# rvp-group/srrg2_slam_interfaces

Hardware: AMD Instinct MI355X
Metric: icp_iterations_per_sec (higher is better)
Workload: dtype f32; 1 GPU; C2: SE(3) point-to-plane AlignerSlice, 100000-pt synthetic cloud pair per GPU, 10 ICP iterations per compute(), gated NN 0.25 m + normal gate, Cauchy 0.05; points=100000, alignments_total=1, all_success=True, last_status=0, last_num_inliers=99432, parallelism=single GPU

## Files before the change

include/srrg2_slam_amd.h:

```cpp
#ifndef SRRG2_SLAM_AMD_H
#define SRRG2_SLAM_AMD_H

#include <stddef.h>
#include <stdint.h>

#ifdef __cplusplus
extern "C" {
#endif

#define SRRG2_AMD_ABI_VERSION 4
#define SRRG2_MAX_SLICES 8


enum srrg2_variable_kind {
  SRRG2_SE2_RIGHT       = 0,
  SRRG2_SE3_EULER_RIGHT = 1,
  SRRG2_SE3_QUAT_RIGHT  = 2
};

enum srrg2_status {
  SRRG2_SUCCESS                    = 0,
  SRRG2_NOT_ENOUGH_CORRESPONDENCES = 1,
  SRRG2_NOT_ENOUGH_INLIERS         = 2,
  SRRG2_FAIL                       = 3
// ... 390 lines not shown
  float   rmax_cap;
  int32_t search_lists;
  int32_t search_team;
  int32_t batch_pipeline;
  int32_t fused_control;
  int32_t reserved_[6];
} srrg2_aligner_tuning;
void srrg2_aligner_default_tuning(srrg2_aligner_tuning* t);
int srrg2_aligner_get_tuning(srrg2_aligner_h h, srrg2_aligner_tuning* t_out);
int srrg2_aligner_set_tuning(srrg2_aligner_h h, const srrg2_aligner_tuning* t);


int srrg2_aligner_profile_enable(srrg2_aligner_h h, int enable);
int srrg2_aligner_profile_get(srrg2_aligner_h h, double* step_kernel_ms, int64_t* step_kernel_launches,
                              int reset);
#define SRRG2_PATH_FUSED_CONTROL 1
#define SRRG2_PATH_ALL_PASSES_FUSED 2
#define SRRG2_PATH_FINAL_WAVE 4
#define SRRG2_PATH_PROLOGUE_IN_PASS 8
#define SRRG2_PATH_ONE_WORKGROUP 16
#define SRRG2_PATH_PRIORS_FUSED 32
int srrg2_aligner_last_compute_path(srrg2_aligner_h h, int32_t* flags_out);

#ifndef SRRG2_DESCRIPTOR_BYTES
#define SRRG2_DESCRIPTOR_BYTES 32
#endif
typedef struct srrg2_descriptor_db* srrg2_descriptor_db_h;
int srrg2_descriptor_db_create(int device, srrg2_descriptor_db_h* out);
int srrg2_descriptor_db_destroy(srrg2_descriptor_db_h h);
int srrg2_descriptor_db_add(srrg2_descriptor_db_h h, const uint8_t* descriptors, const uint8_t* valid, int n,
                            int* index_out);
int srrg2_descriptor_db_size(srrg2_descriptor_db_h h, int* maps, int64_t* descriptors);
int srrg2_descriptor_db_match(srrg2_descriptor_db_h h, const uint8_t* descriptors, const uint8_t* valid, int n,
                              int64_t query_index, float max_distance, uint32_t min_age, int64_t min_matches,
                              int* K_out);
int srrg2_descriptor_db_get_candidates(srrg2_descriptor_db_h h, int32_t* reference, int64_t* num_matches,
                                       int64_t* corr_offsets, int* n_inout);
int srrg2_descriptor_db_get_correspondences(srrg2_descriptor_db_h h, srrg2_correspondence* buf, int64_t* n_inout);
int srrg2_descriptor_db_get_map_counts(srrg2_descriptor_db_h h, int64_t* counts, int* n_inout);
int srrg2_descriptor_db_last_match_ms(srrg2_descriptor_db_h h, double* ms);
int srrg2_descriptor_db_add_scene(srrg2_descriptor_db_h h, srrg2_scene_h scene, int* index_out);
int srrg2_descriptor_db_match_scene(srrg2_descriptor_db_h h, srrg2_scene_h scene, int64_t query_index, float max_distance,
                                    uint32_t min_age, int64_t min_matches, int* K_out);

#ifdef __cplusplus
}
// ... 3 lines not shown
```

srrg2_slam_interfaces_amd/csrc/aligner_host.hip:

```cpp
#include <algorithm>
#include <cmath>
#include <cstdio>
#include <cstdlib>
#include <chrono>
#include <cstring>
#include <string>
#include <vector>

#include "det_math.h"
#include "kernels.h"

#include "host_util.h"

namespace srrg2amd {
thread_local std::string g_err;
int fail(int code, const std::string& msg) {
  g_err = msg;
  return code;
}
}

namespace {

using srrg2amd::DevBuf;
using srrg2amd::fail;

struct Slice {
  srrg2_slice_config cfg;
  DevBuf<float4> fixed_raw, fixed_nrm_raw;
  DevBuf<float4> fixed_sorted, fixed_nrm_sorted;
  DevBuf<int> cell_start, cursor, scan_sums, pos_of;
  DevBuf<unsigned> scalars;
  GridDev grid{};
  DevBuf<int> list_start, list_sums;
  DevBuf<uint4> list_ent;
  DevBuf<uint2> list_box;
  DevBuf<int4> list_offs;
  DevBuf<GridLists> list_hdr;
  GridLists lists_host{};
  bool lists_tried = false;
  int grid_computes = 0;
  int nf          = 0;
  float probe_h = 0.f, probe_ext = 0.f, probe_gate = 0.f, probe_target = 0.f;
  int probe_n   = 0;
  bool has_fixed  = false;
  bool fixed_has_normals = false;
  int alias_of = -1;
  DevBuf<float4> moving, moving_nrm;
  DevBuf<float4> moving_raw, moving_nrm_raw;
  DevBuf<int> ms_counts, ms_cursor, ms_sums;
  DevBuf<unsigned> ms_bb;
  DevBuf<ProblemDev> ms_probs;
  DevBuf<unsigned> pinf;
  int nm_total            = 0;
  bool has_moving         = false;
  bool moving_is_batch    = false;
  bool moving_has_normals = false;
  DevBuf<int> corr_fixed;
// ... 17 lines not shown
  const void* slots_zeroed_at = nullptr;
  int slots_zeroed = 0;
  unsigned* bbox_host = nullptr; size_t bbox_host_cap = 0;
  unsigned bbox_seq = 0;
  bool scalars_self_init = false;
  DevBuf<unsigned> bbox_rows;
  DevBuf<unsigned long long> zbuf;
  DevBuf<int> queue;
  DevBuf<int> qcount;
  float prior_Z[12]{};
  bool has_prior = false;
  void release() {
    if (qprobe_host) (void) hipHostFree(qprobe_host);
    qprobe_host = nullptr;
    qprobe_cap  = 0;
    if (bbox_host) (void) hipHostFree(bbox_host);
    bbox_host     = nullptr;
    bbox_host_cap = 0;
    if (ms_probs_host) (void) hipHostFree(ms_probs_host);
    ms_probs_host     = nullptr;
    ms_probs_host_cap = 0;
    fixed_raw.release(); fixed_nrm_raw.release(); fixed_sorted.release(); fixed_nrm_sorted.release();
    cell_start.release(); cursor.release(); scan_sums.release(); scalars.release(); pos_of.release();
    list_start.release(); list_sums.release(); list_ent.release(); list_box.release(); list_offs.release(); list_hdr.release();
    moving.release(); moving_nrm.release(); pinf.release();
    moving_raw.release(); moving_nrm_raw.release(); ms_counts.release(); ms_cursor.release(); ms_sums.release();
    ms_bb.release(); ms_probs.release();
    corr_fixed.release(); gcorr.release(); gcorr_off.release(); gcorr_stat.release(); prev_n.release(); prev_pos.release(); prev_f.release(); prev_m.release(); corr_resp.release(); corr_stat.release(); partials.release(); zbuf.release(); queue.release(); qcount.release(); bbox_rows.release();
  }
};

}

struct srrg2_aligner_s {
  int kind = 0, dim = 3, dof = 6, tsize = 12, device = 0;
  hipStream_t stream = nullptr;
  static constexpr int MAX_PARTS = 8;
  hipStream_t pstream[MAX_PARTS]{};
  int cu_count          = 256;
  int fused_grid_max    = 130000;
  hipEvent_t ev_staged  = nullptr;
  hipEvent_t ev_records = nullptr;
  bool records_unsynced = false;
  int parts_dirty       = 0;
  int batch_parts       = 0;
  int part_begin[MAX_PARTS + 1]{};
  srrg2_aligner_params params{10, 10, 0, 0};
// ... 381 lines not shown
        const int m = sep(x) + sep(y) + sep(z);
        if (m > CNL_MAX_CLASS || class_bound2(m) > g.gate2_ext) continue;
        offs.push_back(Off{x, y, z, m, x * x + y * y + z * z});
      }
  if ((long long) offs.size() * ((long long) s->nf + s->nf / CNL_ENTRY_MAX + 1) >= (1LL << 31)) return 0;
  std::stable_sort(offs.begin(), offs.end(), [](const Off& p, const Off& q) { return p.cls != q.cls ? p.cls < q.cls : p.c2 < q.c2; });
  std::vector<int4> offs4(offs.size());
  for (size_t k = 0; k < offs.size(); ++k) offs4[k] = make_int4(offs[k].x, offs[k].y, offs[k].z, offs[k].cls);
  GridLists L{};
  L.R   = R;
  L.lnx = g.nx + 2 * R;
  L.lny = g.ny + 2 * R;
  L.lnz = dim == 3 ? g.nz + 2 * R : 1;
  const long long ncell_ll = (long long) L.lnx * L.lny * L.lnz;
  if (ncell_ll > (1LL << 28)) return 0;
  const int ncell = (int) ncell_ll;
  for (int m = 0; m <= CNL_MAX_CLASS; ++m) L.cls_b2[m] = class_bound2(m);
  L.cls_b2[CNL_MAX_CLASS + 1] = 3.0e38f;
  int rc;
  if ((rc = s->list_offs.reserve(offs4.size()))) return rc;
  if ((rc = s->list_start.reserve((size_t) ncell + 1))) return rc;
  if ((rc = s->list_sums.reserve((size_t) srrg2amd::scan_num_blocks(ncell) + 2))) return rc;
  if ((rc = s->list_hdr.reserve(1))) return rc;
  HIP_TRY(hipMemcpyAsync(s->list_offs.p, offs4.data(), offs4.size() * sizeof(int4), hipMemcpyHostToDevice, a->stream));
  HIP_TRY(hipStreamSynchronize(a->stream));
  srrg2amd::launch_cnl_build(g, L, s->list_offs.p, (int) offs4.size(), s->list_start.p, nullptr, nullptr, a->stream);
  int* total_dev = s->list_sums.p + s->list_sums.cap - 1;
  srrg2amd::launch_exclusive_scan(s->list_start.p, ncell, s->list_sums.p, total_dev, a->stream);
  int total = 0;
  HIP_TRY(hipMemcpyAsync(&total, total_dev, sizeof(int), hipMemcpyDeviceToHost, a->stream));
  HIP_TRY(hipStreamSynchronize(a->stream));
  if (total < 0 || (long long) total > max_entries) return 0;
  if (s->list_ent.reserve((size_t) std::max(total, 1) + 8) || s->list_box.reserve((size_t) std::max(s->nf, 1) + 8)) {
    (void) hipGetLastError();
    s->list_ent.release();
    s->list_box.release();
    return 0;
  }
  L.start = s->list_start.p;
  L.ent   = s->list_ent.p;
  srrg2amd::launch_cnl_build(g, L, s->list_offs.p, (int) offs4.size(), s->list_start.p, s->list_box.p, s->list_ent.p, a->stream);
  HIP_TRY(hipMemcpyAsync(s->list_hdr.p, &L, sizeof(L), hipMemcpyHostToDevice, a->stream));
  HIP_TRY(hipGetLastError());
  HIP_TRY(hipStreamSynchronize(a->stream));
  g.lists       = s->list_hdr.p;
  g.list_R      = R;
  s->lists_host = L;
  return 0;
}

void tuning_from_environment(srrg2_aligner_tuning* t) {
  srrg2_aligner_default_tuning(t);
  auto geti = [](const char* name, int32_t& v) {
    if (const char* e = std::getenv(name)) v = (int32_t) std::atoi(e);
  };
  auto getf = [](const char* name, float& v) {
    if (const char* e = std::getenv(name)) v = (float) std::atof(e);
  };
  geti("SRRG2_AMD_TUNE", t->strategy_mask);
  geti("SRRG2_AMD_QPROBE", t->queue_probe_iteration);
  geti("SRRG2_AMD_SMALL_MAX", t->small_max_points);
  geti("SRRG2_AMD_FAST_FROM", t->fast_from_iteration);
  geti("SRRG2_AMD_FAST_PPT", t->fast_points_per_thread);
  geti("SRRG2_AMD_FAST_MIN", t->fast_min_points);
// ... 1944 lines not shown
int srrg2_aligner_profile_enable(srrg2_aligner_h a, int enable) {
  if (!a) return fail(SRRG2_E_INVALID, "profile_enable: null handle");
  a->profile = enable != 0;
  return 0;
}

int srrg2_aligner_profile_get(srrg2_aligner_h a, double* ms, int64_t* launches, int reset) {
  if (!a) return fail(SRRG2_E_INVALID, "profile_get: null handle");
  if (ms) *ms = a->prof_ms;
  if (launches) *launches = a->prof_launches;
  if (reset) {
    a->prof_ms       = 0.0;
    a->prof_launches = 0;
  }
  return 0;
}

int srrg2_aligner_last_compute_path(srrg2_aligner_h a, int32_t* flags_out) {
  if (!a || !flags_out) return fail(SRRG2_E_INVALID, "last_compute_path: null argument");
  *flags_out = a->computed ? a->last_path : 0;
  return 0;
}

}
```

srrg2_slam_interfaces_amd/csrc/device_types.h:

```cpp
#pragma once
#include <hip/hip_runtime.h>
#include <stdint.h>

#include "../../include/srrg2_slam_amd.h"

#define ACC_N 32
#define PARTIAL_SLOTS 32
#define ACC_B 21
#define ACC_CHI_IN 27
#define ACC_CHI_OUT 28
#define ACC_N_IN 29
#define ACC_N_OUT 30
#define ACC_N_CORR 31
#define TERM_WINDOW_MAX 64
#define NO_MATCH 0x7fffffff

__host__ __device__ __forceinline__ constexpr int hidx(int a, int b) {
  return a * 6 - (a * (a - 1)) / 2 + (b - a);
}

struct GridDev {
  float ox, oy, oz;
  float h, inv_h;
  int nx, ny, nz;
  int rmax;
  int rfar_gate;
  float gate2;
  float gate2_ext;
  int n;
  const int* cell_start;
  const float4* pts;
  const float4* nrm;
  const int* pos_of;
  int list_R;
  const struct GridLists* lists;
};
struct GridLists {
  int R;
  int lnx, lny, lnz;
  const int* start;
  const uint4* ent;
  float cls_b2[14];
};
#define CNL_MAX_R 3
#ifndef CNL_ENTRY_MAX
#define CNL_ENTRY_MAX 16
#endif
#define CNL_MAX_CLASS 12

#define PUB_SLICE_GRANULES 64
#define PUB_G_KEXP 24
#define PUB_G_FLAGS 25
#define PUB_G_NSTATS 26
#define PUB_G_WCOUNT 27
#define PUB_G_NPASSES 28
#define PUB_G_X 32
#define PUB_FLAG_STOP 1u
#define PUB_FLAG_PHASE1 2u
#define PUB_FLAG_PRIOR 4u
#define PUB_EPOCH_REPLICAS 8
#define PUB_EPOCH_STRIDE 32
struct CtlParams;
struct FusedCtl {
  unsigned long long* pub;
  unsigned* pub_epoch;
  const CtlParams* ctl;
// ... 150 lines not shown
```

srrg2_slam_interfaces_amd/csrc/kernels.h:

```cpp
#pragma once
#include "device_types.h"

namespace srrg2amd {

void launch_ingest(const float* src, int stride_floats, int n, int dim, float4* dst, unsigned* maxabs_bits,
                   int finite_per_point, hipStream_t s);
void launch_ingest_batch(const float* src, int stride_floats, const ProblemDev* probs, int K, int max_nm, int dim,
                         float4* dst, unsigned* maxabs_bits, int finite_per_point, hipStream_t s);
void launch_bbox(const float4* pts, int n, unsigned* mn, unsigned* mx, int* nvalid, hipStream_t s);
void launch_ingest_bbox(const float* src, int stride_floats, int n, int dim, float4* dst, unsigned* maxabs_bits, unsigned* mn,
                        unsigned* mx, int* nvalid, hipStream_t s, unsigned* ticket, unsigned* host_out, unsigned seq,
                        unsigned* block_out , unsigned* clear_after);
#define INGEST_BBOX_MAX_BLOCKS 512
void launch_grid_count(const GridDev& g, const float4* pts, int n, int* counts, hipStream_t s);
void launch_count_nonzero(const int* counts, int n, int* out, hipStream_t s);
int scan_num_blocks(int n);
void launch_exclusive_scan(int* data, int n, int* block_sums, int* grand_total, hipStream_t s, int* copy = nullptr);
void launch_grid_scatter(const GridDev& g, const float4* pts, const float4* nrm, int n, int* cursor, float4* out_pts,
                         float4* out_nrm, int* pos_of, hipStream_t s);
void launch_cnl_build(const GridDev& g, const GridLists& L, const int4* offs, int noffs, int* list_start, uint2* box_at,
                      uint4* ent, hipStream_t s);
void launch_icp_step_cnl(int dim, bool plane, const SliceDev& S, const GridLists& GL, const ProblemDev* probs,
                         ProblemState* states, int K, int max_nm, int team, hipStream_t s, const CtlParams* init_C = nullptr,
                         const InitInline* init_inl = nullptr, const InitBatch* init_bat = nullptr);
bool launch_msort_local(const float* src, int sf, const float* nsrc, int nsf, const ProblemDev* probs, int K, int dim, int kbits,
                        int aniso, int segments, int max_nm, float4* out_pts, float4* out_nrm, unsigned* maxabs_bits,
                        hipStream_t s);
void launch_msort(const float4* pts, const float4* nrm, const ProblemDev* probs, int K, int max_nm, int kbits, int aniso,
                  unsigned* bb, int* counts, int* cursor, int* scan_sums, int* scan_total, float4* out_pts,
                  float4* out_nrm, hipStream_t s);
void launch_icp_step(int dim, bool plane, const SliceDev& S, const ProblemDev* probs, ProblemState* states, int K,
                     int max_nm, hipStream_t s, const CtlParams* init_C = nullptr, const InitInline* init_inl = nullptr);
void launch_icp_step_tile(int dim, bool plane, const SliceDev& S, const ProblemDev* probs, ProblemState* states, int K,
                          int max_nm, int cap, hipStream_t s);
void launch_icp_step_fast(int dim, bool plane, const SliceDev& S, const ProblemDev* probs, ProblemState* states, int K,
                          int max_nm, int ppt, bool gather, hipStream_t s);
void launch_icp_outputs(int dim, bool plane, const SliceDev& S, const ProblemDev* probs, const ProblemState* states, int K,
                        int max_nm, hipStream_t s);
int icp_step_blocks(int max_nm);
int icp_queue_blocks(int max_nm, int K);
void launch_proj_step_pack(const SliceDev* slices, const ProblemDev* const* probs, int nslices, ProblemState* states, int K,
                           int max_nm, hipStream_t s);
void launch_proj_records(const SliceDev& S0, const SliceDev& S, const ProblemDev* probs0, const ProblemDev* probs,
                         ProblemState* states, int K, int max_nm, bool rebuild, hipStream_t s);
// ... 38 lines not shown
```

srrg2_slam_interfaces_amd/csrc/kernels.hip:

```cpp
#include <cstdlib>
#include <algorithm>

#include "kernels.h"

#include <type_traits>

#include "det_math.h"

#include "device_util.h"

namespace {

#define FX_MAGIC 6755399441055744.0
#define FX_MAGIC_BITS 0x4338000000000000ll
__device__ __forceinline__ long long fx_bits(double biased) { return __double_as_longlong(biased) - FX_MAGIC_BITS; }

__device__ __forceinline__ unsigned long long key_min(unsigned long long a, unsigned long long b) {
  double r;
  asm("v_min_f64 %0, %1, %2" : "=v"(r) : "v"(__longlong_as_double((long long) a)), "v"(__longlong_as_double((long long) b)));
  return (unsigned long long) __double_as_longlong(r);
}

template <int DIM>
__device__ __forceinline__ float cand_d2(const float4 f, float qx, float qy, float qz) {
// ... 454 lines not shown
    }
    wave_lds_sync();
  }
  unsigned long long kmin = key;
#pragma unroll
  for (int off = TW / 2; off >= 1; off >>= 1) {
    const unsigned long long o = __shfl_xor(kmin, off);
    kmin = o < kmin ? o : kmin;
  }
  wpos  = 0;
  wbest = __uint_as_float((unsigned) (kmin >> 32));
  widx  = (int) (unsigned) kmin;
  float v = key == kmin ? lb2 : fminf(lb2, __uint_as_float((unsigned) (key >> 32)));
#pragma unroll
  for (int off = TW / 2; off >= 1; off >>= 1) v = fminf(v, __shfl_xor(v, off));
  wexcl2 = fminf(v, fminf(sr2, bound2_of(max(sr, 0), g.h)));
}

namespace {

#ifndef SRRG2_CNL_REDEAL
#define SRRG2_CNL_REDEAL 0
#endif
#ifdef SRRG2_CNL_STATS
__device__ unsigned long long g_cnl_stats[4 * 16];
#define CNL_STAT(k, v)                                                                                   \
  do {                                                                                                   \
    const unsigned long long v_ = (unsigned long long) (v);    \
    if ((threadIdx.x & 63) == 0) atomicAdd(&g_cnl_stats[(stat_it < 3 ? stat_it : 3) * 16 + (k)], v_);    \
  } while (0)
#else
#define CNL_STAT(k, v) do { } while (0)
#endif
constexpr int CNL_POOL = 512;

struct CnlWave {
  uint2 pool[CNL_POOL];
  unsigned long long key[64];
  unsigned b2[64];
  float q[3][64];
};

template <int DIM>
__device__ __forceinline__ void test_group_glb(const float4* __restrict__ pts, int j, int cnt, float qx, float qy, float qz,
                                               unsigned long long& bkey, float& b2) {
  if (cnt > 0) {
// ... 31 lines not shown
    const int owner = (int) (it.y & 63u);
    int cnt         = have ? (int) (it.y >> 8) : 0;
    int j           = (int) it.x;
    const float qx = w.q[0][owner], qy = w.q[1][owner], qz = DIM == 3 ? w.q[2][owner] : 0.f;
    unsigned long long key = NO_KEY;
    float lb2              = INFINITY;
    while (__any(cnt > 0)) {
      CNL_STAT(8, 1);
      CNL_STAT(9, __popcll(__ballot(cnt > 0)));
      test_group_glb<DIM>(pts, j, cnt, qx, qy, qz, key, lb2);
      j += 4;
      cnt -= 4;
    }
    if (have) {
      const unsigned long long old   = atomicMin(&w.key[owner], key);
      const unsigned long long loser = old > key ? old : key;
      const unsigned l2              = min((unsigned) (loser >> 32), __float_as_uint(lb2));
      atomicMin(&w.b2[owner], l2);
    }
  }
  wave_lds_sync();
}

template <int DIM, int TEAM>
__device__ __forceinline__ void cnl_phase0(const GridDev& g, const GridLists& gl, int lane, bool need, float qx, float qy, float qz,
                                           float r2box, float gfar, unsigned long long& bkey, float& b2, float& L, int& e,
                                           int& eend, int stat_it = 3) {
  const int R  = gl.R;
  const int tl = lane & (TEAM - 1);
  const int cx = cell_coord(qx, g.ox, g.inv_h);
  const int cy = cell_coord(qy, g.oy, g.inv_h);
  const int cz = DIM == 3 ? cell_coord(qz, g.oz, g.inv_h) : 0;
  const int lx = cx + R, ly = cy + R, lz = DIM == 3 ? cz + R : 0;
  const bool inl = need && lx >= 0 && lx < gl.lnx && ly >= 0 && ly < gl.lny && lz >= 0 && lz < gl.lnz;
  e = 0;
  eend = 0;
  if (inl) {
    const int lc = (lz * gl.lny + ly) * gl.lnx + lx;
    e            = gl.start[lc];
    eend         = gl.start[lc + 1];
  }
  bkey = NO_KEY;
  b2   = INFINITY;
  L    = fminf(r2box, gfar);
  {
    const bool p0 = e < eend;
    uint4 h0      = make_uint4(0u, 0u, 0u, 0u);
    if (p0) h0 = gl.ent[e];
    int j = (int) h0.x + 4 * tl, cnt = p0 ? (int) (h0.y & 15u) + 1 - 4 * tl : 0;
    CNL_STAT(10, __popcll(__ballot(need)));
    while (__any(cnt > 0)) {
      CNL_STAT(1, 1);
      CNL_STAT(2, __popcll(__ballot(cnt > 0)));
      test_group_glb<DIM>(g.pts, j, cnt, qx, qy, qz, bkey, b2);
      j += 4 * TEAM;
      cnt -= 4 * TEAM;
    }
#pragma unroll
    for (int off = 1; off < TEAM; off <<= 1) {
      const unsigned long long ok = __shfl_xor(bkey, off);
      const float ob2             = __shfl_xor(b2, off);
      const unsigned long long lo = ok < bkey ? ok : bkey, hi = ok < bkey ? bkey : ok;
      b2   = fminf(fminf(b2, ob2), __uint_as_float((unsigned) (hi >> 32)));
      bkey = lo;
    }
    if (p0) {
      ++e;
      if (key_idx(bkey) != NO_MATCH) {
        const float rb = (sqrtf(key_best(bkey)) + (PAD_CAP + PAD_MIN) * g.h) * 1.00001f;
        L              = fminf(L, rb * rb);
      }
    }
  }
}

template <int DIM, int TEAM>
__device__ __forceinline__ void cnl_phaseAB(const GridDev& g, const GridLists& gl, CnlWave& w, int lane, float qx, float qy,
                                            float qz, unsigned long long& bkey, float& b2, float L, int e, int eend,
                                            int stat_it = 3) {
  const int R  = gl.R;
  const int tl = lane & (TEAM - 1);
  const int owner_lane = lane - tl;
  const float ux0 = (qx - g.ox) * g.inv_h, uy0 = (qy - g.oy) * g.inv_h, uz0 = DIM == 3 ? (qz - g.oz) * g.inv_h : 0.f;
  const int cx = cell_coord(qx, g.ox, g.inv_h);
  const int cy = cell_coord(qy, g.oy, g.inv_h);
  const int cz = DIM == 3 ? cell_coord(qz, g.oz, g.inv_h) : 0;
  if (tl == 0) {
    w.key[lane]  = bkey;
    w.b2[lane]   = __float_as_uint(b2);
    w.q[0][lane] = qx;
    w.q[1][lane] = qy;
    if (DIM == 3) w.q[2][lane] = qz;
  }
  const float Lc  = L * 1.00002f;
  const float Lcc = ((Lc * g.inv_h) * g.inv_h * 1.0001f) * 256.f;
  int mmax = -1;
#pragma unroll
  for (int m = 0; m <= CNL_MAX_CLASS; ++m) mmax += gl.cls_b2[m] <= Lc ? 1 : 0;
  const float fR = (float) R;
  const float mx = 0.011f + fabsf(ux0) * 1e-6f, my = 0.011f + fabsf(uy0) * 1e-6f, mz = 0.011f + fabsf(uz0) * 1e-6f;
  const float ux = ux0 - (float) cx, uy = uy0 - (float) cy, uz = uz0 - (float) cz;
  const float cax = ((fR + ux) + mx) * 16.f, cbx = ((fR + ux) - mx) * 16.f;
  const float cay = ((fR + uy) + my) * 16.f, cby = ((fR + uy) - my) * 16.f;
  const float caz = ((fR + uz) + mz) * 16.f, cbz = ((fR + uz) - mz) * 16.f;
  int pool_n = 0;
  e += 4 * tl;
  CNL_STAT(0, 1);
  CNL_STAT(11, __popcll(__ballot(e < eend)));
  while (__any(e < eend)) {
    CNL_STAT(3, 1);
    CNL_STAT(4, __popcll(__ballot(e < eend)));
    uint4 hd[4];
#pragma unroll
    for (int k = 0; k < 4; ++k) {
      hd[k] = make_uint4(0u, 0xf0u, 0u, 0u);
      if (e + k < eend) hd[k] = gl.ent[e + k];
    }
    bool stop = e >= eend;
#pragma unroll
    for (int k = 0; k < 4; ++k) {
      const unsigned code = hd[k].y;
      stop = stop || (int) ((code >> 4) & 15u) > mmax;
      const unsigned blo = hd[k].z, bhi = hd[k].w;
      const float lx_ = (float) (blo & 255u), ly_ = (float) ((blo >> 8) & 255u);
      const float hx_ = (float) (bhi & 255u), hy_ = (float) ((bhi >> 8) & 255u);
      const float tx = fmaxf(fmaxf(lx_ - cax, cbx - hx_), 0.f);
      const float ty = fmaxf(fmaxf(ly_ - cay, cby - hy_), 0.f);
      float d2c      = __fmaf_rn(ty, ty, tx * tx);
      if (DIM == 3) {
        const float lz_ = (float) ((blo >> 16) & 255u), hz_ = (float) ((bhi >> 16) & 255u);
        const float tz  = fmaxf(fmaxf(lz_ - caz, cbz - hz_), 0.f);
        d2c             = __fmaf_rn(tz, tz, d2c);
      }
      const bool surv             = !stop && !(d2c > Lcc);
      const unsigned long long bm = __ballot(surv);
      if (surv) {
        const int slot = pool_n + (int) __builtin_amdgcn_mbcnt_hi((unsigned) (bm >> 32), __builtin_amdgcn_mbcnt_lo((unsigned) bm, 0u));
        w.pool[slot]   = make_uint2(hd[k].x, (unsigned) owner_lane | (((code & 15u) + 1u) << 8));
      }
      pool_n += __popcll(bm);
    }
    e = stop ? eend : min(e + 4 * TEAM, eend);
    if (pool_n > CNL_POOL - 256) {
      cnl_drain_pool<DIM>(g.pts, w, lane, pool_n, stat_it);
      pool_n = 0;
    }
  }
  cnl_drain_pool<DIM>(g.pts, w, lane, pool_n, stat_it);
  bkey = w.key[owner_lane];
  b2   = __uint_as_float(w.b2[owner_lane]);
}

template <int DIM, int TEAM>
__device__ __forceinline__ void cnl_search(const GridDev& g, const GridLists& gl, CnlWave& w, int lane, bool need, float qx,
                                           float qy, float qz, float r2box, float gfar, unsigned long long& bkey, float& b2,
                                           float& L, int stat_it = 3) {
  int e, eend;
  cnl_phase0<DIM, TEAM>(g, gl, lane, need, qx, qy, qz, r2box, gfar, bkey, b2, L, e, eend, stat_it);
  cnl_phaseAB<DIM, TEAM>(g, gl, w, lane, qx, qy, qz, bkey, b2, L, e, eend, stat_it);
}

}

template <int DIM, bool PLANE>
__device__ __forceinline__ void finish_point(const SliceDev& S, const float* T, int rk, float thr, float kk, double scale,
                                             bool inrange, bool active, int gi, int oi, const float4 p, float qx, float qy,
                                             float qz, float best, int bidx, int bpos, float excl, bool kept,
                                             const float4 kept_f, const float4 kept_n, const float4 early_nm, bool have_nm,
                                             long long (&acc)[ACC_N]) {
  constexpr int D    = DIM == 3 ? 6 : 3;
  constexpr int ROWS = PLANE ? 1 : DIM;
  const GridDev& g   = S.grid;
  int match     = -1;
  float resp    = 0.f;
  uint8_t fstat = SRRG2_FACTOR_SUPPRESSED;
  float4 fm     = make_float4(0.f, 0.f, 0.f, __int_as_float(NO_MATCH));
  float4 nf     = make_float4(0.f, 0.f, 0.f, 0.f);
  if (inrange) {
    if (active) {
      bool found = bidx != NO_MATCH && best <= g.gate2;
      if (!kept && bidx != NO_MATCH) bpos = g.pos_of[bidx];
      if (bidx != NO_MATCH && (PLANE || S.use_normal_gate))
// ... 2603 lines not shown
        excl    = pm * 0.9999999f - dl * 1.00001f;
      } else {
        const float pad = fminf(2.f * dl, PAD_CAP * g.h) + PAD_MIN * g.h;
        const float rr  = (d1 + pad) * 1.00001f;
        r2box           = fminf(rr * rr, gfar);
      }
    } else if (use_prior && !has_prev && pm > 0.f) {
      float px, py, pz;
      transform_point<DIM>(Tprev, p, px, py, pz);
      const float ex = qx - px, ey = qy - py, ez = qz - pz;
      const float dl = sqrtf((ex * ex + ey * ey) + ez * ez);
      if (sqrtf(g.gate2) * 1.00001f + dl * 1.00001f < pm * 0.99999f) {
        skipped = true;
        excl    = pm * 0.9999999f - dl * 1.00001f;
      }
    }
  }
  const bool need = active && !skipped;
  if constexpr (TEAM == 1 && SRRG2_CNL_REDEAL != 0) {
    __shared__ unsigned long long wcnt[NW];
    unsigned long long k0;
    float b20, L;
    int e, eend;
    cnl_phase0<DIM, 1>(g, GL, lane, need, qx, qy, qz, r2box, gfar, k0, b20, L, e, eend, S.fc.epoch);
    const float est = (float) (eend - e) * fminf(L * (1.f / gfar), 1.f);
    const int cls   = (est > 4.f ? 1 : 0) + (est > 8.f ? 1 : 0) + (est > 16.f ? 1 : 0);
    const unsigned long long m1 = __ballot(cls == 1), m2 = __ballot(cls == 2), m3 = __ballot(cls == 3);
    const unsigned long long m0 = ~(m1 | m2 | m3);
    if (lane == 0)
      wcnt[wid] = (unsigned long long) __popcll(m0) | ((unsigned long long) __popcll(m1) << 16) |
                  ((unsigned long long) __popcll(m2) << 32) | ((unsigned long long) __popcll(m3) << 48);
    __syncthreads();
    int slot;
    {
      unsigned long long tot = 0ull, before = 0ull;
#pragma unroll
      for (int k = 0; k < NW; ++k) {
        const unsigned long long c = wcnt[k];
        tot += c;
        before += k < wid ? c : 0ull;
      }
      const unsigned long long mm = cls == 0 ? m0 : cls == 1 ? m1 : cls == 2 ? m2 : m3;
      const unsigned long long below = tot & ((1ull << (16 * cls)) - 1ull);
      slot = (int) ((below & 0xffffull) + ((below >> 16) & 0xffffull) + ((below >> 32) & 0xffffull)) +
             (int) ((before >> (16 * cls)) & 0xffffull) +
             (int) __builtin_amdgcn_mbcnt_hi((unsigned) (mm >> 32), __builtin_amdgcn_mbcnt_lo((unsigned) mm, 0u));
    }
    {
      float* tw = reinterpret_cast<float*>(wlds[slot >> 6].pool);
      const int sl = slot & 63;
      tw[sl]       = qx;
      tw[64 + sl]  = qy;
      tw[128 + sl] = qz;
      tw[192 + sl] = L;
      tw[256 + sl] = __int_as_float(e);
      tw[320 + sl] = __int_as_float(eend);
    }
    __syncthreads();
    {
      const float* tr = reinterpret_cast<const float*>(wlds[wid].pool);
      const float ax = tr[lane], ay = tr[64 + lane], az = tr[128 + lane], aL = tr[192 + lane];
      const int ae = __float_as_int(tr[256 + lane]), aend = __float_as_int(tr[320 + lane]);
      wave_lds_sync();
      unsigned long long ka = NO_KEY;
      float ba              = INFINITY;
      cnl_phaseAB<DIM, 1>(g, GL, wlds[wid], lane, ax, ay, az, ka, ba, aL, ae, aend, S.fc.epoch);
    }
    __syncthreads();
    if (need) {
      const unsigned long long ka = wlds[slot >> 6].key[slot & 63];
      const float ba              = __uint_as_float(wlds[slot >> 6].b2[slot & 63]);
      const unsigned long long lo = ka < k0 ? ka : k0, hi = ka < k0 ? k0 : ka;
      const float b2              = fminf(fminf(b20, ba), __uint_as_float((unsigned) (hi >> 32)));
      best = key_best(lo);
      bidx = key_idx(lo);
      excl = sqrtf(fminf(b2, fminf(L, g.gate2_ext))) * 0.99999f;
    }
  } else if (__any(need)) {
    unsigned long long bkey;
    float b2, L;
    cnl_search<DIM, TEAM>(g, GL, wlds[wid], lane, need, qx, qy, qz, r2box, gfar, bkey, b2, L, S.fc.epoch);
    if (need) {
      best = key_best(bkey);
      bidx = key_idx(bkey);
      excl = sqrtf(fminf(b2, fminf(L, g.gate2_ext))) * 0.99999f;
    }
  }
  constexpr int D    = DIM == 3 ? 6 : 3;
  constexpr int ROWS = PLANE ? 1 : DIM;
// ... 1889 lines not shown
```

srrg2_slam_interfaces_amd/csrc/kernels_prep.hip:

```cpp
#include <cstdlib>
#include "kernels.h"

#include "device_util.h"

__global__ void k_ingest(const float* __restrict__ src, int stride_floats, int n, int dim, float4* __restrict__ dst,
                         unsigned* __restrict__ maxabs_bits, int finite_per_point) {
  int i      = blockIdx.x * blockDim.x + threadIdx.x;
  float amax = 0.f;
  if (i < n) {
    const float* p = src + (size_t) i * stride_floats;
    float x = p[0], y = p[1], z = dim == 3 ? p[2] : 0.f;
    dst[i] = make_float4(x, y, z, 0.f);
    bool ok = finite3(x, y, z);
    if (finite_per_point) {
      if (ok) amax = fmaxf(fmaxf(fabsf(x), fabsf(y)), fabsf(z));
    } else {
      if (isfinite(x)) amax = fmaxf(amax, fabsf(x));
      if (isfinite(y)) amax = fmaxf(amax, fabsf(y));
      if (isfinite(z)) amax = fmaxf(amax, fabsf(z));
    }
  }
#pragma unroll
  for (int off = 32; off >= 1; off >>= 1) amax = fmaxf(amax, __shfl_xor(amax, off));
  if (!maxabs_bits) return;
// ... 433 lines not shown
      const int cc[3] = {cx, cy, cz};
#pragma unroll
      for (int d = 0; d < 3; ++d) {
        const float u = (v[d] - o[d]) * g.inv_h;
        const float f = u - (float) cc[d];
        int a = (int) floorf(f * 16.f), b = a + 1;
        if (!(f >= 0.f) || !(f < 1.f)) {
          a = 0;
          b = 16;
        }
        a = a < 0 ? 0 : (a > 15 ? 15 : a);
        b = b < 1 ? 1 : (b > 16 ? 16 : b);
        lo[d] = a < lo[d] ? a : lo[d];
        hi[d] = b > hi[d] ? b : hi[d];
      }
    }
    box_at[s] = make_uint2((unsigned) lo[0] | ((unsigned) lo[1] << 8) | ((unsigned) lo[2] << 16),
                           (unsigned) hi[0] | ((unsigned) hi[1] << 8) | ((unsigned) hi[2] << 16));
  }
}

__global__ __launch_bounds__(256) void k_cnl_fill(GridDev g, GridLists L, const int4* __restrict__ offs, int noffs, int ncell,
                                                  const int* __restrict__ list_start, const uint2* __restrict__ box_at,
                                                  uint4* __restrict__ ent) {
  const int lc = blockIdx.x * blockDim.x + threadIdx.x;
  if (lc >= ncell) return;
  int at       = list_start[lc];
  const int R  = L.R;
  for (int k = 0; k < noffs; ++k) {
    const int4 o = offs[k];
    int cnt;
    const int c = cnl_target_cell(g, L, lc, o, cnt);
    if (cnt <= 0) continue;
    const unsigned code = ((unsigned) o.w << 4) | ((unsigned) (o.x + R) << 8) | ((unsigned) (o.y + R) << 16) |
                          ((unsigned) (o.z + R) << 24);
    int start = g.cell_start[c];
    const unsigned base = ((unsigned) (o.x + R) * 16u) | (((unsigned) (o.y + R) * 16u) << 8) | (((unsigned) (o.z + R) * 16u) << 16);
    while (cnt > 0) {
      const int m    = cnt < CNL_ENTRY_MAX ? cnt : CNL_ENTRY_MAX;
      const uint2 bx = box_at[start];
      ent[at++]      = make_uint4((unsigned) start, code | (unsigned) (m - 1), base + bx.x, base + bx.y);
      start += m;
      cnt -= m;
    }
  }
}

__device__ __forceinline__ unsigned spread3(unsigned v) {
  v = (v | (v << 8)) & 0x0000f00fu;
  v = (v | (v << 4)) & 0x000c30c3u;
  v = (v | (v << 2)) & 0x00249249u;
  return v;
}

__device__ __forceinline__ unsigned spread2(unsigned v) {
  v = (v | (v << 8)) & 0x00ff00ffu;
  v = (v | (v << 4)) & 0x0f0f0f0fu;
  v = (v | (v << 2)) & 0x33333333u;
  v = (v | (v << 1)) & 0x55555555u;
  return v;
}

struct KeySpec {
  float mn[3], scale[3];
  int b[3];
  int ia, ib, ic;
};

// ... 364 lines not shown
  launch_exclusive_scan(cell_start, total_cells, scan_sums, scan_total, s, cursor);
  hipLaunchKernelGGL(k_pairs_localize, dim3(pairs_blocks(max_cells + 1), K), dim3(256), 0, s, grids, fprobs);
  if (max_nf > 0)
    hipLaunchKernelGGL(k_pairs_grid_scatter, dim3(pairs_blocks(max_nf), K), dim3(256), 0, s, grids, fprobs, pts, nrm, cell_start,
                       cursor, out_pts, out_nrm, pos_of);
}

void launch_msort(const float4* pts, const float4* nrm, const ProblemDev* probs, int K, int max_nm, int kbits, int aniso,
                  unsigned* bb, int* counts, int* cursor, int* scan_sums, int* scan_total, float4* out_pts,
                  float4* out_nrm, hipStream_t s) {
  if (K <= 0 || max_nm <= 0) return;
  int bx = (max_nm + 255) / 256;
  if (bx > 1024) bx = 1024;
  dim3 grid(bx, K);
  if (((long long) K << kbits) > 0x3fffffffLL) return;
  const int ncell = K << kbits;
  hipLaunchKernelGGL(k_msort_bbox, dim3(bx < 32 ? bx : 32, K), dim3(256), 0, s, pts, probs, bb);
  hipLaunchKernelGGL(k_msort_count, grid, dim3(256), 0, s, pts, probs, bb, kbits, aniso, counts);
  launch_exclusive_scan(counts, ncell, scan_sums, scan_total, s, cursor);
  hipLaunchKernelGGL(k_msort_scatter, grid, dim3(256), 0, s, pts, nrm, probs, bb, kbits, aniso, cursor, out_pts, out_nrm);
}

void launch_cnl_build(const GridDev& g, const GridLists& L, const int4* offs, int noffs, int* list_start, uint2* box_at,
                      uint4* ent, hipStream_t s) {
  const int ncell = L.lnx * L.lny * L.lnz;
  if (ncell <= 0 || noffs <= 0) return;
  if (!ent) {
    hipLaunchKernelGGL(k_cnl_count, dim3((ncell + 255) / 256), dim3(256), 0, s, g, L, offs, noffs, ncell, list_start);
  } else {
    const int gcell = g.nx * g.ny * g.nz;
    hipLaunchKernelGGL(k_cnl_boxes, dim3((gcell + 255) / 256), dim3(256), 0, s, g, gcell, box_at);
    hipLaunchKernelGGL(k_cnl_fill, dim3((ncell + 255) / 256), dim3(256), 0, s, g, L, offs, noffs, ncell, list_start, box_at, ent);
  }
}

bool launch_msort_local(const float* src, int sf, const float* nsrc, int nsf, const ProblemDev* probs, int K, int dim, int kbits,
                        int aniso, int segments, int max_nm, float4* out_pts, float4* out_nrm, unsigned* maxabs_bits,
                        hipStream_t s) {
  if (kbits > 15) return false;
  if (K <= 0) return true;
  const int seg_env = segments;
  int G = seg_env > 0 ? seg_env : (K >= 256 ? 1 : (K >= 64 ? 2 : (128 / K < 8 ? 128 / K : 8)));
  if (seg_env <= 0 && K <= 4) {
    const int by_size = max_nm / 3072, room = 64 / K;
    G = G > (by_size < room ? by_size : room) ? G : (by_size < room ? by_size : room);
  }
  if (G < 1) G = 1;
  if (G > 1) {
    if (!aniso) kbits = kbits < 12 ? kbits : 12;
    (void) hipMemsetAsync(maxabs_bits, 0, (size_t) K * sizeof(unsigned), s);
  }
  if (aniso && kbits > 12 && max_nm / G < 8192) kbits = 12;
  const size_t lds = sizeof(int) << kbits;
  static bool attr_ok = hipFuncSetAttribute(reinterpret_cast<const void*>(k_msort_local),
                                            hipFuncAttributeMaxDynamicSharedMemorySize, (int) (sizeof(int) << 15)) == hipSuccess;
// ... 11 lines not shown
```

Baseline: 59470 iterations/s.

## Precompute per-cell class boundary table to bound cell-list scans in NN search

The cell-list build now also writes, for each list cell, a packed row of per-distance-class entry counts, with a wide flag for lists longer than 255 entries. The search phase uses this row to compute up front where the scan ends for the current radius class. The old per-entry class-stop check is kept only as a fallback loop for wide cells. This removes that check from the common path and lets header loads skip the sentinel handling. It also adds optional compile-time prefetching of header groups (off by default), costs one extra uint4 load per query plus extra LDS traffic in the team path, and adds a debug read-back API.

```diff
diff --git a/include/srrg2_slam_amd.h b/include/srrg2_slam_amd.h
--- a/include/srrg2_slam_amd.h
+++ b/include/srrg2_slam_amd.h
@@ -436,6 +436,9 @@
 #define SRRG2_PATH_PRIORS_FUSED 32
 int srrg2_aligner_last_compute_path(srrg2_aligner_h h, int32_t* flags_out);
 
+int srrg2_cell_lists_read(srrg2_aligner_h h, int slice_idx, int32_t* num_lists, int32_t* num_entries, int32_t* start,
+                          uint32_t* entries, uint8_t* boundaries);
+
 #ifndef SRRG2_DESCRIPTOR_BYTES
 #define SRRG2_DESCRIPTOR_BYTES 32
 #endif
diff --git a/srrg2_slam_interfaces_amd/csrc/aligner_host.hip b/srrg2_slam_interfaces_amd/csrc/aligner_host.hip
--- a/srrg2_slam_interfaces_amd/csrc/aligner_host.hip
+++ b/srrg2_slam_interfaces_amd/csrc/aligner_host.hip
@@ -34,6 +34,7 @@
   GridDev grid{};
   DevBuf<int> list_start, list_sums;
   DevBuf<uint4> list_ent;
+  DevBuf<uint4> list_bnd;
   DevBuf<uint2> list_box;
   DevBuf<int4> list_offs;
   DevBuf<GridLists> list_hdr;
@@ -97,7 +98,7 @@
     ms_probs_host_cap = 0;
     fixed_raw.release(); fixed_nrm_raw.release(); fixed_sorted.release(); fixed_nrm_sorted.release();
     cell_start.release(); cursor.release(); scan_sums.release(); scalars.release(); pos_of.release();
-    list_start.release(); list_sums.release(); list_ent.release(); list_box.release(); list_offs.release(); list_hdr.release();
+    list_start.release(); list_sums.release(); list_ent.release(); list_bnd.release(); list_box.release(); list_offs.release(); list_hdr.release();
     moving.release(); moving_nrm.release(); pinf.release();
     moving_raw.release(); moving_nrm_raw.release(); ms_counts.release(); ms_cursor.release(); ms_sums.release();
     ms_bb.release(); ms_probs.release();
@@ -525,9 +526,10 @@
   if ((rc = s->list_start.reserve((size_t) ncell + 1))) return rc;
   if ((rc = s->list_sums.reserve((size_t) srrg2amd::scan_num_blocks(ncell) + 2))) return rc;
   if ((rc = s->list_hdr.reserve(1))) return rc;
+  if ((rc = s->list_bnd.reserve((size_t) ncell))) return rc;
   HIP_TRY(hipMemcpyAsync(s->list_offs.p, offs4.data(), offs4.size() * sizeof(int4), hipMemcpyHostToDevice, a->stream));
   HIP_TRY(hipStreamSynchronize(a->stream));
-  srrg2amd::launch_cnl_build(g, L, s->list_offs.p, (int) offs4.size(), s->list_start.p, nullptr, nullptr, a->stream);
+  srrg2amd::launch_cnl_build(g, L, s->list_offs.p, (int) offs4.size(), s->list_start.p, nullptr, nullptr, nullptr, a->stream);
   int* total_dev = s->list_sums.p + s->list_sums.cap - 1;
   srrg2amd::launch_exclusive_scan(s->list_start.p, ncell, s->list_sums.p, total_dev, a->stream);
   int total = 0;
@@ -542,7 +544,9 @@
   }
   L.start = s->list_start.p;
   L.ent   = s->list_ent.p;
-  srrg2amd::launch_cnl_build(g, L, s->list_offs.p, (int) offs4.size(), s->list_start.p, s->list_box.p, s->list_ent.p, a->stream);
+  L.bnd   = s->list_bnd.p;
+  srrg2amd::launch_cnl_build(g, L, s->list_offs.p, (int) offs4.size(), s->list_start.p, s->list_box.p, s->list_ent.p, s->list_bnd.p,
+                             a->stream);
   HIP_TRY(hipMemcpyAsync(s->list_hdr.p, &L, sizeof(L), hipMemcpyHostToDevice, a->stream));
   HIP_TRY(hipGetLastError());
   HIP_TRY(hipStreamSynchronize(a->stream));
@@ -2533,4 +2537,27 @@
   return 0;
 }
 
-}
+int srrg2_cell_lists_read(srrg2_aligner_h a, int slice_idx, int32_t* num_lists, int32_t* num_entries, int32_t* start,
+                          uint32_t* entries, uint8_t* boundaries) {
+  if (!a || !num_lists || !num_entries) return fail(SRRG2_E_INVALID, "cell_lists_read: null argument");
+  if (slice_idx < 0 || slice_idx >= (int) a->slices.size()) return fail(SRRG2_E_INVALID, "cell_lists_read: no such slice");
+  int rc;
+  if ((rc = set_device(a))) return rc;
+  const Slice* s = a->slices[(size_t) slice_idx];
+  *num_lists     = 0;
+  *num_entries   = 0;
+  if (s->grid.list_R <= 0) return 0;
+  const GridLists& L = s->lists_host;
+  const int ncell    = L.lnx * L.lny * L.lnz;
+  HIP_TRY(hipStreamSynchronize(a->stream));
+  int total = 0;
+  HIP_TRY(hipMemcpy(&total, L.start + ncell, sizeof(int), hipMemcpyDeviceToHost));
+  *num_lists   = ncell;
+  *num_entries = total;
+  if (start) HIP_TRY(hipMemcpy(start, L.start, ((size_t) ncell + 1) * sizeof(int), hipMemcpyDeviceToHost));
+  if (entries && total > 0) HIP_TRY(hipMemcpy(entries, L.ent, (size_t) total * sizeof(uint4), hipMemcpyDeviceToHost));
+  if (boundaries) HIP_TRY(hipMemcpy(boundaries, L.bnd, (size_t) ncell * sizeof(uint4), hipMemcpyDeviceToHost));
+  return 0;
+}
+
+}
diff --git a/srrg2_slam_interfaces_amd/csrc/device_types.h b/srrg2_slam_interfaces_amd/csrc/device_types.h
--- a/srrg2_slam_interfaces_amd/csrc/device_types.h
+++ b/srrg2_slam_interfaces_amd/csrc/device_types.h
@@ -41,7 +41,10 @@
   const int* start;
   const uint4* ent;
   float cls_b2[14];
-};
+  const uint4* bnd;
+};
+#define CNL_BND_MAX 255
+#define CNL_BND_WIDE 0x80000000u
 #define CNL_MAX_R 3
 #ifndef CNL_ENTRY_MAX
 #define CNL_ENTRY_MAX 16
diff --git a/srrg2_slam_interfaces_amd/csrc/kernels.h b/srrg2_slam_interfaces_amd/csrc/kernels.h
--- a/srrg2_slam_interfaces_amd/csrc/kernels.h
+++ b/srrg2_slam_interfaces_amd/csrc/kernels.h
@@ -19,7 +19,7 @@
 void launch_grid_scatter(const GridDev& g, const float4* pts, const float4* nrm, int n, int* cursor, float4* out_pts,
                          float4* out_nrm, int* pos_of, hipStream_t s);
 void launch_cnl_build(const GridDev& g, const GridLists& L, const int4* offs, int noffs, int* list_start, uint2* box_at,
-                      uint4* ent, hipStream_t s);
+                      uint4* ent, uint4* bnd, hipStream_t s);
 void launch_icp_step_cnl(int dim, bool plane, const SliceDev& S, const GridLists& GL, const ProblemDev* probs,
                          ProblemState* states, int K, int max_nm, int team, hipStream_t s, const CtlParams* init_C = nullptr,
                          const InitInline* init_inl = nullptr, const InitBatch* init_bat = nullptr);
diff --git a/srrg2_slam_interfaces_amd/csrc/kernels.hip b/srrg2_slam_interfaces_amd/csrc/kernels.hip
--- a/srrg2_slam_interfaces_amd/csrc/kernels.hip
+++ b/srrg2_slam_interfaces_amd/csrc/kernels.hip
@@ -500,6 +500,9 @@
 #ifndef SRRG2_CNL_REDEAL
 #define SRRG2_CNL_REDEAL 0
 #endif
+#ifndef SRRG2_CNL_AHEAD
+#define SRRG2_CNL_AHEAD 0
+#endif
 #ifdef SRRG2_CNL_STATS
 __device__ unsigned long long g_cnl_stats[4 * 16];
 #define CNL_STAT(k, v)                                                                                   \
@@ -577,10 +580,10 @@
   wave_lds_sync();
 }
 
-template <int DIM, int TEAM>
+template <int DIM, int TEAM, bool PRE>
 __device__ __forceinline__ void cnl_phase0(const GridDev& g, const GridLists& gl, int lane, bool need, float qx, float qy, float qz,
                                            float r2box, float gfar, unsigned long long& bkey, float& b2, float& L, int& e,
-                                           int& eend, int stat_it = 3) {
+                                           int& eend, uint4& row, uint4 (&hpre)[4], int stat_it = 3) {
   const int R  = gl.R;
   const int tl = lane & (TEAM - 1);
   const int cx = cell_coord(qx, g.ox, g.inv_h);
@@ -590,10 +593,12 @@
   const bool inl = need && lx >= 0 && lx < gl.lnx && ly >= 0 && ly < gl.lny && lz >= 0 && lz < gl.lnz;
   e = 0;
   eend = 0;
+  row  = make_uint4(0u, 0u, 0u, 0u);
   if (inl) {
     const int lc = (lz * gl.lny + ly) * gl.lnx + lx;
     e            = gl.start[lc];
     eend         = gl.start[lc + 1];
+    row          = gl.bnd[lc];
   }
   bkey = NO_KEY;
   b2   = INFINITY;
@@ -602,6 +607,15 @@
     const bool p0 = e < eend;
     uint4 h0      = make_uint4(0u, 0u, 0u, 0u);
     if (p0) h0 = gl.ent[e];
+    if constexpr (PRE) {
+      const int pa = e + 1 + 4 * tl;
+#pragma unroll
+      for (int k = 0; k < 4; ++k) hpre[k] = make_uint4(0u, 0u, 0u, 0u);
+      if (pa < eend) {
+#pragma unroll
+        for (int k = 0; k < 4; ++k) hpre[k] = gl.ent[pa + k];
+      }
+    }
     int j = (int) h0.x + 4 * tl, cnt = p0 ? (int) (h0.y & 15u) + 1 - 4 * tl : 0;
     CNL_STAT(10, __popcll(__ballot(need)));
     while (__any(cnt > 0)) {
@@ -629,10 +643,40 @@
   }
 }
 
-template <int DIM, int TEAM>
+struct CnlBall {
+  float cax, cbx, cay, cby, caz, cbz, Lcc;
+};
+template <int DIM>
+__device__ __forceinline__ void cnl_test_headers(CnlWave& w, const CnlBall& c, const uint4 (&hd)[4], int nvalid, int owner_lane,
+                                                 int& pool_n) {
+#pragma unroll
+  for (int k = 0; k < 4; ++k) {
+    const unsigned code = hd[k].y;
+    const unsigned blo = hd[k].z, bhi = hd[k].w;
+    const float lx_ = (float) (blo & 255u), ly_ = (float) ((blo >> 8) & 255u);
+    const float hx_ = (float) (bhi & 255u), hy_ = (float) ((bhi >> 8) & 255u);
+    const float tx = fmaxf(fmaxf(lx_ - c.cax, c.cbx - hx_), 0.f);
+    const float ty = fmaxf(fmaxf(ly_ - c.cay, c.cby - hy_), 0.f);
+    float d2c      = __fmaf_rn(ty, ty, tx * tx);
+    if (DIM == 3) {
+      const float lz_ = (float) ((blo >> 16) & 255u), hz_ = (float) ((bhi >> 16) & 255u);
+      const float tz  = fmaxf(fmaxf(lz_ - c.caz, c.cbz - hz_), 0.f);
+      d2c             = __fmaf_rn(tz, tz, d2c);
+    }
+    const bool surv             = k < nvalid && !(d2c > c.Lcc);
+    const unsigned long long bm = __ballot(surv);
+    if (surv) {
+      const int slot = pool_n + (int) __builtin_amdgcn_mbcnt_hi((unsigned) (bm >> 32), __builtin_amdgcn_mbcnt_lo((unsigned) bm, 0u));
+      w.pool[slot]   = make_uint2(hd[k].x, (unsigned) owner_lane | (((code & 15u) + 1u) << 8));
+    }
+    pool_n += __popcll(bm);
+  }
+}
+
+template <int DIM, int TEAM, bool PRE>
 __device__ __forceinline__ void cnl_phaseAB(const GridDev& g, const GridLists& gl, CnlWave& w, int lane, float qx, float qy,
                                             float qz, unsigned long long& bkey, float& b2, float L, int e, int eend,
-                                            int stat_it = 3) {
+                                            const uint4 row, uint4 (&hn)[4], int stat_it = 3) {
   const int R  = gl.R;
   const int tl = lane & (TEAM - 1);
   const int owner_lane = lane - tl;
@@ -648,54 +692,77 @@
     if (DIM == 3) w.q[2][lane] = qz;
   }
   const float Lc  = L * 1.00002f;
-  const float Lcc = ((Lc * g.inv_h) * g.inv_h * 1.0001f) * 256.f;
+  CnlBall c;
+  c.Lcc = ((Lc * g.inv_h) * g.inv_h * 1.0001f) * 256.f;
   int mmax = -1;
 #pragma unroll
   for (int m = 0; m <= CNL_MAX_CLASS; ++m) mmax += gl.cls_b2[m] <= Lc ? 1 : 0;
   const float fR = (float) R;
   const float mx = 0.011f + fabsf(ux0) * 1e-6f, my = 0.011f + fabsf(uy0) * 1e-6f, mz = 0.011f + fabsf(uz0) * 1e-6f;
   const float ux = ux0 - (float) cx, uy = uy0 - (float) cy, uz = uz0 - (float) cz;
-  const float cax = ((fR + ux) + mx) * 16.f, cbx = ((fR + ux) - mx) * 16.f;
-  const float cay = ((fR + uy) + my) * 16.f, cby = ((fR + uy) - my) * 16.f;
-  const float caz = ((fR + uz) + mz) * 16.f, cbz = ((fR + uz) - mz) * 16.f;
+  c.cax = ((fR + ux) + mx) * 16.f, c.cbx = ((fR + ux) - mx) * 16.f;
+  c.cay = ((fR + uy) + my) * 16.f, c.cby = ((fR + uy) - my) * 16.f;
+  c.caz = ((fR + uz) + mz) * 16.f, c.cbz = ((fR + uz) - mz) * 16.f;
   int pool_n = 0;
-  e += 4 * tl;
+  const bool wide = (row.w & CNL_BND_WIDE) != 0u;
+  int wend;
+  {
+    const int mm        = mmax < 0 ? 0 : mmax;
+    const unsigned word = mm < 4 ? row.x : (mm < 8 ? row.y : (mm < 12 ? row.z : row.w));
+    const int len       = mmax < 0 ? 0 : (int) ((word >> ((mm & 3) * 8)) & 255u);
+    wend                = min(e - 1 + len, eend);
+  }
+  int p = e + 4 * tl;
+  if (wide) wend = p;
   CNL_STAT(0, 1);
-  CNL_STAT(11, __popcll(__ballot(e < eend)));
-  while (__any(e < eend)) {
+  CNL_STAT(11, __popcll(__ballot(p < wend)));
+  auto load_group = [&](int at, uint4 (&h)[4]) {
+    if (at < wend) {
+#pragma unroll
+      for (int k = 0; k < 4; ++k) h[k] = gl.ent[at + k];
+    }
+  };
+  constexpr bool AHEAD = SRRG2_CNL_AHEAD >= 1;
+  if constexpr (AHEAD && !PRE) load_group(p, hn);
+  while (__any(p < wend)) {
     CNL_STAT(3, 1);
-    CNL_STAT(4, __popcll(__ballot(e < eend)));
+    CNL_STAT(4, __popcll(__ballot(p < wend)));
     uint4 hd[4];
+    const int nvalid = wend - p;
+    if constexpr (AHEAD) {
+#pragma unroll
+      for (int k = 0; k < 4; ++k) hd[k] = hn[k];
+      p += 4 * TEAM;
+      load_group(p, hn);
+    } else {
+#pragma unroll
+      for (int k = 0; k < 4; ++k) hd[k] = make_uint4(0u, 0u, 0u, 0u);
+      load_group(p, hd);
+      p += 4 * TEAM;
+    }
+    cnl_test_headers<DIM>(w, c, hd, nvalid, owner_lane, pool_n);
+    if (pool_n > CNL_POOL - 256) {
+      cnl_drain_pool<DIM>(g.pts, w, lane, pool_n, stat_it);
+      pool_n = 0;
+    }
+  }
+  int ew = wide ? e + 4 * tl : eend;
+  while (__any(ew < eend)) {
+    uint4 hd[4];
+    bool stop = ew >= eend;
+    int nvalid = 0;
 #pragma unroll
     for (int k = 0; k < 4; ++k) {
       hd[k] = make_uint4(0u, 0xf0u, 0u, 0u);
-      if (e + k < eend) hd[k] = gl.ent[e + k];
-    }
-    bool stop = e >= eend;
+      if (ew + k < eend) hd[k] = gl.ent[ew + k];
+    }
 #pragma unroll
     for (int k = 0; k < 4; ++k) {
-      const unsigned code = hd[k].y;
-      stop = stop || (int) ((code >> 4) & 15u) > mmax;
-      const unsigned blo = hd[k].z, bhi = hd[k].w;
-      const float lx_ = (float) (blo & 255u), ly_ = (float) ((blo >> 8) & 255u);
-      const float hx_ = (float) (bhi & 255u), hy_ = (float) ((bhi >> 8) & 255u);
-      const float tx = fmaxf(fmaxf(lx_ - cax, cbx - hx_), 0.f);
-      const float ty = fmaxf(fmaxf(ly_ - cay, cby - hy_), 0.f);
-      float d2c      = __fmaf_rn(ty, ty, tx * tx);
-      if (DIM == 3) {
-        const float lz_ = (float) ((blo >> 16) & 255u), hz_ = (float) ((bhi >> 16) & 255u);
-        const float tz  = fmaxf(fmaxf(lz_ - caz, cbz - hz_), 0.f);
-        d2c             = __fmaf_rn(tz, tz, d2c);
-      }
-      const bool surv             = !stop && !(d2c > Lcc);
-      const unsigned long long bm = __ballot(surv);
-      if (surv) {
-        const int slot = pool_n + (int) __builtin_amdgcn_mbcnt_hi((unsigned) (bm >> 32), __builtin_amdgcn_mbcnt_lo((unsigned) bm, 0u));
-        w.pool[slot]   = make_uint2(hd[k].x, (unsigned) owner_lane | (((code & 15u) + 1u) << 8));
-      }
-      pool_n += __popcll(bm);
-    }
-    e = stop ? eend : min(e + 4 * TEAM, eend);
+      stop = stop || (int) ((hd[k].y >> 4) & 15u) > mmax;
+      nvalid += stop ? 0 : 1;
+    }
+    cnl_test_headers<DIM>(w, c, hd, nvalid, owner_lane, pool_n);
+    ew = stop ? eend : min(ew + 4 * TEAM, eend);
     if (pool_n > CNL_POOL - 256) {
       cnl_drain_pool<DIM>(g.pts, w, lane, pool_n, stat_it);
       pool_n = 0;
@@ -710,9 +777,11 @@
 __device__ __forceinline__ void cnl_search(const GridDev& g, const GridLists& gl, CnlWave& w, int lane, bool need, float qx,
                                            float qy, float qz, float r2box, float gfar, unsigned long long& bkey, float& b2,
                                            float& L, int stat_it = 3) {
+  constexpr bool PRE = SRRG2_CNL_AHEAD >= 2;
   int e, eend;
-  cnl_phase0<DIM, TEAM>(g, gl, lane, need, qx, qy, qz, r2box, gfar, bkey, b2, L, e, eend, stat_it);
-  cnl_phaseAB<DIM, TEAM>(g, gl, w, lane, qx, qy, qz, bkey, b2, L, e, eend, stat_it);
+  uint4 row, hn[4] = {};
+  cnl_phase0<DIM, TEAM, PRE>(g, gl, lane, need, qx, qy, qz, r2box, gfar, bkey, b2, L, e, eend, row, hn, stat_it);
+  cnl_phaseAB<DIM, TEAM, PRE>(g, gl, w, lane, qx, qy, qz, bkey, b2, L, e, eend, row, hn, stat_it);
 }
 
 }
@@ -3362,7 +3431,8 @@
     unsigned long long k0;
     float b20, L;
     int e, eend;
-    cnl_phase0<DIM, 1>(g, GL, lane, need, qx, qy, qz, r2box, gfar, k0, b20, L, e, eend, S.fc.epoch);
+    uint4 row, hn[4] = {};
+    cnl_phase0<DIM, 1, false>(g, GL, lane, need, qx, qy, qz, r2box, gfar, k0, b20, L, e, eend, row, hn, S.fc.epoch);
     const float est = (float) (eend - e) * fminf(L * (1.f / gfar), 1.f);
     const int cls   = (est > 4.f ? 1 : 0) + (est > 8.f ? 1 : 0) + (est > 16.f ? 1 : 0);
     const unsigned long long m1 = __ballot(cls == 1), m2 = __ballot(cls == 2), m3 = __ballot(cls == 3);
@@ -3395,16 +3465,22 @@
       tw[192 + sl] = L;
       tw[256 + sl] = __int_as_float(e);
       tw[320 + sl] = __int_as_float(eend);
+      tw[384 + sl] = __uint_as_float(row.x);
+      tw[448 + sl] = __uint_as_float(row.y);
+      tw[512 + sl] = __uint_as_float(row.z);
+      tw[576 + sl] = __uint_as_float(row.w);
     }
     __syncthreads();
     {
       const float* tr = reinterpret_cast<const float*>(wlds[wid].pool);
       const float ax = tr[lane], ay = tr[64 + lane], az = tr[128 + lane], aL = tr[192 + lane];
       const int ae = __float_as_int(tr[256 + lane]), aend = __float_as_int(tr[320 + lane]);
+      const uint4 arow = make_uint4(__float_as_uint(tr[384 + lane]), __float_as_uint(tr[448 + lane]), __float_as_uint(tr[512 + lane]),
+                                    __float_as_uint(tr[576 + lane]));
       wave_lds_sync();
       unsigned long long ka = NO_KEY;
       float ba              = INFINITY;
-      cnl_phaseAB<DIM, 1>(g, GL, wlds[wid], lane, ax, ay, az, ka, ba, aL, ae, aend, S.fc.epoch);
+      cnl_phaseAB<DIM, 1, false>(g, GL, wlds[wid], lane, ax, ay, az, ka, ba, aL, ae, aend, arow, hn, S.fc.epoch);
     }
     __syncthreads();
     if (need) {
diff --git a/srrg2_slam_interfaces_amd/csrc/kernels_prep.hip b/srrg2_slam_interfaces_amd/csrc/kernels_prep.hip
--- a/srrg2_slam_interfaces_amd/csrc/kernels_prep.hip
+++ b/srrg2_slam_interfaces_amd/csrc/kernels_prep.hip
@@ -479,16 +479,28 @@
 
 __global__ __launch_bounds__(256) void k_cnl_fill(GridDev g, GridLists L, const int4* __restrict__ offs, int noffs, int ncell,
                                                   const int* __restrict__ list_start, const uint2* __restrict__ box_at,
-                                                  uint4* __restrict__ ent) {
+                                                  uint4* __restrict__ ent, uint4* __restrict__ bnd) {
   const int lc = blockIdx.x * blockDim.x + threadIdx.x;
   if (lc >= ncell) return;
-  int at       = list_start[lc];
-  const int R  = L.R;
+  const int at0 = list_start[lc];
+  int at        = at0;
+  const int R   = L.R;
+  unsigned row[4] = {0u, 0u, 0u, 0u};
+  int next_cls    = 0;
+  auto close_classes = [&](int upto) {
+    const unsigned n = (unsigned) (at - at0 < CNL_BND_MAX ? at - at0 : CNL_BND_MAX);
+    for (; next_cls < upto; ++next_cls) {
+      const unsigned v = n << ((next_cls & 3) * 8);
+#pragma unroll
+      for (int w = 0; w < 4; ++w) row[w] |= (next_cls >> 2) == w ? v : 0u;
+    }
+  };
   for (int k = 0; k < noffs; ++k) {
     const int4 o = offs[k];
     int cnt;
     const int c = cnl_target_cell(g, L, lc, o, cnt);
     if (cnt <= 0) continue;
+    close_classes(o.w);
     const unsigned code = ((unsigned) o.w << 4) | ((unsigned) (o.x + R) << 8) | ((unsigned) (o.y + R) << 16) |
                           ((unsigned) (o.z + R) << 24);
     int start = g.cell_start[c];
@@ -501,6 +513,9 @@
       cnt -= m;
     }
   }
+  close_classes(CNL_MAX_CLASS + 1);
+  if (at - at0 > CNL_BND_MAX) row[3] |= CNL_BND_WIDE;
+  bnd[lc] = make_uint4(row[0], row[1], row[2], row[3]);
 }
 
 __device__ __forceinline__ unsigned spread3(unsigned v) {
@@ -911,7 +926,7 @@
 }
 
 void launch_cnl_build(const GridDev& g, const GridLists& L, const int4* offs, int noffs, int* list_start, uint2* box_at,
-                      uint4* ent, hipStream_t s) {
+                      uint4* ent, uint4* bnd, hipStream_t s) {
   const int ncell = L.lnx * L.lny * L.lnz;
   if (ncell <= 0 || noffs <= 0) return;
   if (!ent) {
@@ -919,7 +934,7 @@
   } else {
     const int gcell = g.nx * g.ny * g.nz;
     hipLaunchKernelGGL(k_cnl_boxes, dim3((gcell + 255) / 256), dim3(256), 0, s, g, gcell, box_at);
-    hipLaunchKernelGGL(k_cnl_fill, dim3((ncell + 255) / 256), dim3(256), 0, s, g, L, offs, noffs, ncell, list_start, box_at, ent);
+    hipLaunchKernelGGL(k_cnl_fill, dim3((ncell + 255) / 256), dim3(256), 0, s, g, L, offs, noffs, ncell, list_start, box_at, ent, bnd);
   }
 }
 
```

Result: faster. 60500 iterations/s (median of 5 runs) (+1.7%).
